# IntelLabs/bayesian-torch

Hardware: AMD Instinct MI355X
Metric: MC-samples/sec (Bayesian-ResNet18, 224^2, bs=64) (higher is better)
Workload: dtype bf16

## Files before the change

### bayesian_torch_amd/csrc/btx_api.hip

```cpp
#include <hip/hip_runtime.h>
#include <math.h>
#include <string.h>
#include "../../include/btx.h"
#include <stdlib.h>
#include "btx_contract.h"
#include "btx_rng.h"
#include "btx_presample.h"

using namespace btx;

static int contract_fwd_impl(int kind, const BtxGeom* g, const void* x, const float* mu_w, const float* rho_w,
                             const float* mu_b, const float* rho_b, void* out, const BtxRng* rng, const BtxNoise* noise,
                             int act_dtype, int prec, uint32_t flags, void* ws, size_t ws_bytes, void* stream,
                             const BtxEpilogue* ep, const BtxLanes* ln) {
  if (!g || !x || !mu_w || !rho_w || !out || !rng) return BTX_E_NULL;
  const int lanes = ln ? ln->n : 1;
  if ((mu_b == nullptr) != (rho_b == nullptr)) return BTX_E_NULL;
  const uintptr_t al = (uintptr_t)x | (uintptr_t)mu_w | (uintptr_t)rho_w | (uintptr_t)out |
                       (uintptr_t)(noise && noise->eps_w ? noise->eps_w : nullptr) |
                       (uintptr_t)(ep && ep->residual ? ep->residual : nullptr);
  FwdSel sel;
  int rc = select_fwd(kind, g, act_dtype, prec, flags, (al & 15) != 0, noise, ep, &sel);
  if (rc) return rc;
  const Plan& pl = sel.pl;
// ... 48 lines not shown
  {
    const long long in_elems = (long long)g->NB * g->D * g->H * g->W * g->C;
    const long long xb = in_elems * (act_dtype == BTX_ACT_BF16 ? 2 : 4), wb = (long long)g->N * pl.K * 4;
    p.x_bytes = xb < 0xffffffffLL ? (uint32_t)xb : 0xffffffffu;
    p.w_bytes = wb < 0xffffffffLL ? (uint32_t)wb : 0xffffffffu;
  }

  p.fd_inner = make_fastdiv((uint32_t)(pl.ntiles * g->groups * pl.ksplits)); p.fd_ksplits = make_fastdiv((uint32_t)pl.ksplits);
  p.fd_ntiles = make_fastdiv((uint32_t)pl.ntiles); p.fd_rtiles = make_fastdiv(1u);
  p.fd_mtiles = make_fastdiv((uint32_t)(pl.mtiles > 0 ? pl.mtiles : 1));
  {
    const double w_b = (prec == BTX_PREC_BF16 ? 2.0 : 4.0) * (double)g->N * pl.K * (kind == BTX_KIND_FLIPOUT ? 2 : 1);
    p.wg_order = (uses_tiles(sel.family) && pl.mtiles > 1 && w_b >= WG_MAJOR_MIB * 1048576.0) ? 1 : 0;
  }
  p.fd_Wo = make_fastdiv((uint32_t)pl.Wo); p.fd_Ho = make_fastdiv((uint32_t)pl.Ho); p.fd_Do = make_fastdiv((uint32_t)pl.Do);
  if (uses_tiles(sel.family)) {
    p.wt = sampled_w ? (void*)sampled_w : (void*)((unsigned char*)ws + sel.wt_off);
    p.wt_ready = sampled_w ? 1 : 0;
    p.wt_bytes = (uint32_t)sel.wt_all;
    p.wt_delta_off = (uint32_t)sel.wt_one;
    p.lane_wt = (long long)sel.wt_one;
    p.lane_wt_delta = (kind == BTX_KIND_FLIPOUT) ? 1 : 0;
  }
  hipStream_t st = (hipStream_t)stream;
  typedef int (*LaunchFn)(int, const ContractParams&, int, hipStream_t);
  auto launch = [&](LaunchFn f32, LaunchFn bf16, LaunchFn x3) {
    return (prec == BTX_PREC_BF16 ? bf16 : prec == BTX_PREC_BF16X3 ? x3 : f32)(kind, p, pl.nwg * lanes, st);
  };
  switch (sel.family) {
    case BTX_FAMILY_STEM_POOL: {
      const StemPoolPlan& spp = sel.spp;
      p.pt_R = spp.PB; p.pt_rtiles = spp.bands; p.pt_Rp = spp.Rp; p.pt_astage = spp.astage; p.st_sbytes = spp.sbytes;
      p.pt_lds = spp.lds; p.pt_PP = spp.patch_bytes; p.sp_Hq = spp.Hq; p.sp_Wq = spp.Wq;
      p.fd_rtiles = make_fastdiv((uint32_t)spp.bands);
      rc = launch_stem_pool_bf16(kind, p, pl.nwg * lanes, st);
      break;
    }
    case BTX_FAMILY_STEM: {
      const StemPlan& stp = sel.stp;
      p.pt_R = stp.R; p.pt_Rp = stp.Rp; p.pt_rtiles = stp.rtiles; p.pt_nw = stp.nw; p.pt_astage = stp.astage;
      p.st_sbytes = stp.sbytes; p.pt_lds = stp.lds; p.pt_PP = stp.patch_bytes;
      p.fd_rtiles = make_fastdiv((uint32_t)stp.rtiles);
      rc = launch(launch_contract_stem_f32, launch_contract_stem_bf16, launch_contract_stem_x3);
      break;
    }
    case BTX_FAMILY_PATCH:
    case BTX_FAMILY_TAPS:
    case BTX_FAMILY_TAPS2: {
      const PatchPlan& pt = sel.pt;
      p.pt_G = pt.G; p.pt_R = pt.R; p.pt_Rp = pt.Rp; p.pt_Wp = pt.Wp; p.pt_PP = pt.PP; p.pt_NI = pt.NI;
      p.fd_ptWp = make_fastdiv((uint32_t)pt.Wp); p.fd_ptRp = make_fastdiv((uint32_t)pt.Rp); p.fd_ptR = make_fastdiv((uint32_t)pt.R);
      p.fd_rtiles = make_fastdiv((uint32_t)pt.rtiles);
      p.pt_rtiles = pt.rtiles; p.pt_nw = pt.nw; p.pt_astage = pt.astage; p.pt_lds = pt.lds;
      p.pt_taps = pt.taps; p.pt_kg = pt.kg; p.pt_lds_g = pt.lds_g;
      p.pt_wide = (pt.taps == 33 || pt.taps == 332) ? pt.wide : 0;
      if (p.pt_wide) {
        p.fd_ntiles = make_fastdiv((uint32_t)(pl.ntiles / 2));
        p.fd_inner = make_fastdiv((uint32_t)((pl.ntiles / 2) * g->groups * pl.ksplits));
      }
      p.pt_tall = pt.tall; p.pt_P = pt.P; p.pt_Wt = pt.Wt; p.pt_ncs = pt.ncs;
      p.fd_P = make_fastdiv((uint32_t)pt.P); p.fd_Wt = make_fastdiv((uint32_t)pt.Wt); p.fd_ncs = make_fastdiv((uint32_t)pt.ncs);
      rc = launch(launch_contract_patch_f32, launch_contract_patch_bf16, launch_contract_patch_x3);
      break;
    }
    case BTX_FAMILY_GEMM8:
      p.pt_rtiles = sel.g8_pairs;
// ... 139 lines not shown
```

### bayesian_torch_amd/csrc/btx_contract.h

```cpp
#pragma once
#include <hip/hip_runtime.h>
#include <stdint.h>
#include "btx_rng.h"
#include "btx_plan.h"

typedef __attribute__((ext_vector_type(8))) __bf16 bf16x8;
typedef __attribute__((ext_vector_type(4))) __bf16 bf16x4;
typedef __attribute__((ext_vector_type(4))) float f32x4;
typedef __attribute__((ext_vector_type(8))) float f32x8;
typedef __attribute__((ext_vector_type(16))) float f32x16;
typedef __attribute__((ext_vector_type(4))) uint32_t u32x4;
typedef __attribute__((ext_vector_type(2))) uint32_t u32x2;

namespace btx {

constexpr int NTHREADS = 512;
constexpr int ACTS_OFF = 0;
constexpr int SIGN_OFF = NG * BM * 16;
constexpr int WMU_OFF = SIGN_OFF + NG * BM * 4;
constexpr int WDL_OFF = WMU_OFF + NG * BN * 16;
constexpr int STAGE_BYTES = WDL_OFF + NG * BN * 16;
constexpr int LDS_BYTES = 2 * STAGE_BYTES;

struct FastDiv {
// ... 37 lines not shown
  int NB, D, H, W, C, Cg;
  int Do, Ho, Wo, N, Ng;
  int KD, KH, KW;
  int sd, sh, sw, pd, ph, pw, dd, dh, dw;
  int M, K;
  int mtiles, ntiles, groups, ksplits, kper;
  int transposed;
  int pointwise;
  uint32_t seed_lo, seed_hi, sample, layer;
  const uint32_t* sample_ptr;
  uint32_t kin_a, kin_b, kout_a, kout_b;
  const float* ep_scale;
  const float* ep_shift;
  const void* ep_res;
  int ep_relu;
  int out_bf16;
  int sign_unaligned;
  uint32_t x_bytes, w_bytes;
  int pt_G, pt_R, pt_Rp, pt_Wp, pt_PP, pt_NI, pt_rtiles;
  FastDiv fd_Wo, fd_Ho, fd_Do, fd_ptWp, fd_ptRp, fd_ptR;
  FastDiv fd_inner, fd_ksplits, fd_ntiles, fd_Cg, fd_KW, fd_KH, fd_rtiles;
  FastDiv fd_mtiles;
  int swap_signs;
  int par_major, par_Mq, par_Mqp, par_Hh, par_Wh;
  FastDiv fd_par_Mqp, fd_par_Hh, fd_par_Wh;
  FastDiv fd_sd, fd_sh, fd_sw;
  int wg_order;
  int pt_nw, pt_astage, pt_lds;
  int pt_kg;
  int pt_lds_g;
  int pt_taps;
  int pt_wide;
  int sp_Hq, sp_Wq;
  int st_sbytes;
  void* wt;
  uint32_t wt_bytes, wt_delta_off;
  int wt_ready;
  int pt_tall, pt_P, pt_Wt, pt_ncs;
  FastDiv fd_P, fd_Wt, fd_ncs;
  int lanes, lane_nwg;
  FastDiv fd_lane_nwg;
  long long lane_x, lane_out, lane_res, lane_wt, lane_partial;
  int lane_wt_delta;
  int reverse;
};

__device__ __forceinline__ uint32_t sample_word_scalar(const uint32_t* ptr) {
  return *(const __attribute__((address_space(4))) uint32_t*)(uintptr_t)ptr;
}

__device__ __forceinline__ int xcd_logical() {
  const int nwg = gridDim.x, L = blockIdx.x;
  const int q = nwg >> 3, r = nwg & 7, xcd = L & 7, slot = L >> 3;
  return (xcd < r ? xcd * (q + 1) : r * (q + 1) + (xcd - r) * q) + slot;
}

__device__ __forceinline__ ContractParams lane_view(const ContractParams& q, int& logical) {
  ContractParams p = q;
  if (q.reverse) logical = (int)gridDim.x - 1 - logical;
  if (q.lanes > 1) {
    uint32_t lane, loc;
    fdivmod((uint32_t)logical, q.fd_lane_nwg, (uint32_t)q.lane_nwg, lane, loc);
    logical = (int)loc;
    const long long l = (long long)lane;
    p.x = (const unsigned char*)q.x + l * q.lane_x;
    p.out = (unsigned char*)q.out + l * q.lane_out;
// ... 682 lines not shown
```

### bayesian_torch_amd/csrc/btx_contract_stempool.h

```cpp
#pragma once
#include <type_traits>
#include "btx_contract.h"
#include "btx_contract_dma.h"
#include "btx_epilogue.h"
#include "btx_mma.h"
#include "btx_presample.h"

namespace btx {

constexpr int SP_NB = 1;
constexpr int SP_HROWS = 2;
constexpr int SP_LROWS = 3;
constexpr int SP_MAXST = 7;

typedef __attribute__((ext_vector_type(8))) short i16x8;

template <bool RELU>
__device__ __forceinline__ u32x4 sp_max8(const u32x4 a, const u32x4 b) {
  if constexpr (RELU) {
    return __builtin_bit_cast(u32x4, __builtin_elementwise_max(__builtin_bit_cast(i16x8, a), __builtin_bit_cast(i16x8, b)));
  } else {
    u32x4 r;
#pragma unroll
    for (int d = 0; d < 4; ++d) {
// ... 28 lines not shown
      }
}

template <int KIND>
__global__ __launch_bounds__(512, 2) void stem_pool_kernel(const ContractParams pk) {
  int logical = xcd_logical();
  const ContractParams p = lane_view(pk, logical);
  constexpr int G = 8, BK = NG * G;
  extern __shared__ __attribute__((aligned(16))) unsigned char smem[];
#define SP_BARRIER() asm volatile("s_waitcnt lgkmcnt(0)\n\ts_barrier" ::: "memory")
  const RngLive rl = rng_live<KIND>(p);

  const int tid = threadIdx.x;
  int lane = tid & 63;
  int l31 = lane & 31;
  int h = lane >> 5;
  const int wave = __builtin_amdgcn_readfirstlane(tid >> 6);
  const int grp = wave >> 2, w4 = wave & 3;
  int gtid = tid & 255;

  uint32_t u_rest, u_ntile, u_img, u_band;
  fdivmod((uint32_t)logical, p.fd_ntiles, (uint32_t)p.ntiles, u_rest, u_ntile);
  fdivmod(u_rest, p.fd_rtiles, (uint32_t)p.pt_rtiles, u_img, u_band);
  const int ntile = (int)u_ntile, img = (int)u_img, band = (int)u_band;

  const int PB = p.pt_R;
  const int P0 = band * PB;
  const int c0 = 2 * P0 - 1;
  const int Hq = p.sp_Hq, Wq = p.sp_Wq, Wo = p.Wo, Ho = p.Ho;
  const int NH = min(PB, Hq - P0) + 1;
  const int RowE = p.W * p.C;
  const int nstages = p.K / BK;
  const int spr = p.Cg / BK;
  const int W_OFF = 0, A_OFF = nstages * DW_STAGE, X_OFF = A_OFF + 2 * p.pt_astage;
  const int S_OFF = X_OFF + (KIND == 1 ? p.pt_astage : 0), R_OFF = S_OFF + 2 * p.st_sbytes;
  const int row_b = Wo * 128;
  const int C_OFF = R_OFF + SP_HROWS * row_b;
  float* const ba_lds = (float*)(smem + R_OFF + SP_LROWS * row_b);
  const int NINF_OFF = R_OFF + SP_LROWS * row_b + 4 * BN * 4;
  if (threadIdx.x < 8) *(uint32_t*)(smem + NINF_OFF + 4 * threadIdx.x) = threadIdx.x < 4 ? 0x80008000u : 0xff80ff80u;

  const __amdgpu_buffer_rsrc_t x_rsrc = __builtin_amdgcn_make_buffer_rsrc((void*)p.x, 0, p.x_bytes, 0x00020000);
  const __amdgpu_buffer_rsrc_t wt_rsrc = __builtin_amdgcn_make_buffer_rsrc((void*)p.wt, 0, p.wt_bytes, 0x00020000);

  {
    constexpr int PER = (KIND == 1) ? 8 : 4;
    const uint32_t w_tile = (uint32_t)ntile * (uint32_t)(p.K / G) * 1024u + (uint32_t)lane * 16u;
    const int npc = nstages * PER;
    for (int i = wave; i < npc; i += 8) {
      const int st = i / PER, r = i % PER;
      const uint32_t src = w_tile + (uint32_t)st * (uint32_t)NG * 1024u + (uint32_t)(r & 3) * 1024u +
                           (r >= 4 ? p.wt_delta_off : 0u);
      dma16(wt_rsrc, src, smem + W_OFF + st * DW_STAGE + (r >= 4 ? 4096 : 0) + (r & 3) * 1024);
    }
  }
  auto tile_base_e = [&](int u) __attribute__((always_inline)) {
    return (img * p.H + (c0 + SP_HROWS * u) * p.sh) * RowE;
  };
  auto issue_patch = [&](int u, int wi, int nw) __attribute__((always_inline)) {
    const uint32_t base_b = (uint32_t)tile_base_e(u) * 2u;
    unsigned char* dst = smem + A_OFF + (u & 1) * p.pt_astage;
    const int npieces = p.pt_astage >> 10;
    for (int i = wi; i < npieces; i += nw) {
      const uint32_t o = (uint32_t)i * 1024u + (uint32_t)lane * 16u;
      dma16(x_rsrc, o < (uint32_t)p.pt_PP ? base_b + o : DMA_OOB, dst + i * 1024);
    }
  };
  auto write_signs = [&](int u, int ti, int nt) __attribute__((always_inline)) {
    if constexpr (KIND == 1) {
      const int word0 = tile_base_e(u) >> 5;
      const int nwords = p.st_sbytes >> 2;
      unsigned char* ss = smem + S_OFF + (u & 1) * p.st_sbytes;
      for (int w = ti; w < nwords; w += nt)
        *(uint32_t*)(ss + w * 4) = btx_sign_word((uint32_t)(word0 + w), rl.kin_a, rl.kin_b);
    }
  };
  auto build_signed = [&](int u) __attribute__((always_inline)) {
    if constexpr (KIND == 1) {
      const int base_e = tile_base_e(u);
      const int word0 = base_e >> 5;
      const unsigned char* raw = smem + A_OFF + (u & 1) * p.pt_astage;
      const unsigned char* ss = smem + S_OFF + (u & 1) * p.st_sbytes;
      unsigned char* dst = smem + X_OFF;
      const int nchunks = p.pt_PP >> 4;
      constexpr int SP_CPY = 5;
      if (nchunks <= SP_CPY * 256) {
        u32x4 v[SP_CPY];
        uint32_t w[SP_CPY];
        int ci[SP_CPY];
#pragma unroll
        for (int k = 0; k < SP_CPY; ++k) {
          ci[k] = min(gtid + 256 * k, nchunks - 1);
          v[k] = *(const u32x4*)(raw + ci[k] * 16);
          w[k] = *(const uint32_t*)(ss + (((base_e + 8 * ci[k]) >> 5) - word0) * 4);
        }
#pragma unroll
        for (int k = 0; k < SP_CPY; ++k) {
          const int e = base_e + 8 * ci[k];
          const uint32_t ws = w[k] << (((uint32_t)e >> 3 & 3u) * 4u);
#pragma unroll
          for (int d = 0; d < 4; ++d) v[k][d] ^= (ws << d) & 0x80008000u;
        }
#pragma unroll
        for (int k = 0; k < SP_CPY; ++k) *(u32x4*)(dst + ci[k] * 16) = v[k];
        return;
      }
      for (int i = gtid; i < nchunks; i += 256) {
        u32x4 v = *(const u32x4*)(raw + i * 16);
        const int e = base_e + 8 * i;
        const uint32_t w = *(const uint32_t*)(ss + ((e >> 5) - word0) * 4);
        const uint32_t ws = w << (((uint32_t)e >> 3 & 3u) * 4u);
#pragma unroll
        for (int d = 0; d < 4; ++d) v[d] ^= (ws << d) & 0x80008000u;
        *(u32x4*)(dst + i * 16) = v;
      }
    }
  };
  issue_patch(0, wave, 8);
  write_signs(0, tid, 512);
  {
    const bool has_bias = p.mu_b != nullptr;
    const bool has_aff = (p.ep_scale != nullptr) || (p.ep_shift != nullptr);
    ep_fill_constants<KIND>(p, rl, ba_lds, tid, ntile, 0, has_bias, has_aff);
  }
  const bool has_bias = p.mu_b != nullptr;
  const bool has_aff = (p.ep_scale != nullptr) || (p.ep_shift != nullptr);
  const bool relu = p.ep_relu != 0;

  int eo[2];
  int st_off[2];
  uint32_t st_orow[2];
#pragma unroll
  for (int mi = 0; mi < 2; ++mi) {
    const int pl = w4 * 64 + mi * 32 + l31;
    const bool ok = pl < 2 * Wo;
    const int plc = ok ? pl : 0;
    const int r = plc >= Wo ? 1 : 0;
    const int col = plc - r * Wo;
    eo[mi] = (r * p.sh * RowE + col * p.sw * p.C) * 2;
    st_off[mi] = ok ? R_OFF + r * row_b + col * 128 + (((col >> 1) & 7) << 4) + h * 8 : -1;
    st_orow[mi] = (uint32_t)(((img * Ho + c0 + r) * Wo + col) * p.N + ntile * BN);
  }
  int pool_coff[2][3];
#pragma unroll
  for (int j = 0; j < 2; ++j)
#pragma unroll
    for (int k = 0; k < 3; ++k) {
      const int pc = (gtid + 256 * j) >> 3, col = 2 * pc - 1 + k;
      pool_coff[j][k] = (pc < Wq && col >= 0 && col < Wo) ? col * 128 + (((gtid & 7) ^ ((col >> 1) & 7)) << 4) : -1;
    }
  int carry_off[4];
#pragma unroll
  for (int j = 0; j < 4; ++j) {
    const int col = (gtid + 256 * j) >> 3;
    carry_off[j] = col < Wo ? col * 128 + (((gtid & 7) ^ ((col >> 1) & 7)) << 4) : -1;
  }
  const __amdgpu_buffer_rsrc_t out_rsrc = __builtin_amdgcn_make_buffer_rsrc(
      p.out, 0, (uint32_t)((size_t)p.NB * Hq * Wq * p.N * 2), 0x00020000);

  f32x16 accm[2][2], accd[2][2];

  auto run_pass = [&](const unsigned char* abase, int woff, f32x16 (&acc)[2][2], int bs0, int bs1, auto mia_tag)
                      __attribute__((always_inline)) {
    constexpr int MIA = decltype(mia_tag)::value;
    int l_j = 0, l_row = 0, l_b = 0;
    auto advance_load = [&]() __attribute__((always_inline)) {
      l_b += BK * 2;
      if (++l_j == spr) { l_j = 0; l_row += RowE * 2; l_b = l_row; }
    };
    auto load = [&](SpFrag& f, int s) __attribute__((always_inline)) {
      const unsigned char* as = abase + l_b;
      const unsigned char* ws = smem + W_OFF + s * DW_STAGE + woff;
#pragma unroll
      for (int kk = 0; kk < NG / 2; ++kk) {
        const int row = 2 * kk + h;
#pragma unroll
        for (int mi = 0; mi < MIA; ++mi) f.a[kk][mi] = *(const u32x4*)(as + eo[mi] + row * 16);
#pragma unroll
        for (int ni = 0; ni < 2; ++ni) f.w[kk][ni] = *(const u32x4*)(ws + (row * BN + ni * 32 + l31) * 16);
      }
      advance_load();
    };
    int nb = 0;
    SpFrag fa, fb;
    load(fa, 0);
    auto iter = [&](int s, SpFrag& cur, SpFrag& nxt, auto zero_tag) __attribute__((always_inline)) {
      if (s == bs0 || s == bs1) { SP_BARRIER(); ++nb; }
      if (s + 1 < nstages) load(nxt, s + 1);
      sp_mma<MIA, decltype(zero_tag)::value>(cur, acc);
    };
    iter(0, fa, fb, std::true_type{});
    int s = 1;
    for (; s + 1 < nstages; s += 2) {
      iter(s, fb, fa, std::false_type{});
      iter(s + 1, fa, fb, std::false_type{});
    }
    if (s < nstages) iter(s, fb, fa, std::false_type{});
    return nb;
  };
  auto run_pass3 = [&](const unsigned char* abase, int woff, f32x16 (&acc)[2][2], int bs0, int bs1) __attribute__((always_inline)) {
    int l_j = 0, l_row = 0, l_b = 0, l_s = 0;
    auto req = [&](SpFrag& f, auto i_tag) __attribute__((always_inline)) {
      constexpr int i = decltype(i_tag)::value, kk = i >> 2, j = i & 3;
      const int row = 2 * kk + h;
      if constexpr (j < 2) f.a[kk][j] = *(const u32x4*)(abase + l_b + eo[j] + row * 16);
      else f.w[kk][j - 2] = *(const u32x4*)(smem + W_OFF + l_s * DW_STAGE + woff + (row * BN + (j - 2) * 32 + l31) * 16);
    };
    auto advance = [&]() __attribute__((always_inline)) {
      ++l_s;
      l_b += BK * 2;
      if (++l_j == spr) { l_j = 0; l_row += RowE * 2; l_b = l_row; }
    };
    auto mma_half = [&](const SpFrag& f, auto kk_tag, auto zero_tag) __attribute__((always_inline)) {
      constexpr int kk = decltype(kk_tag)::value;
      constexpr bool ZERO = decltype(zero_tag)::value;
#pragma unroll
      for (int mi = 0; mi < 2; ++mi)
#pragma unroll
        for (int ni = 0; ni < 2; ++ni) {
          const f32x16 zc = {0.f, 0.f, 0.f, 0.f, 0.f, 0.f, 0.f, 0.f, 0.f, 0.f, 0.f, 0.f, 0.f, 0.f, 0.f, 0.f};
          acc[mi][ni] = __builtin_amdgcn_mfma_f32_32x32x16_bf16(__builtin_bit_cast(bf16x8, f.w[kk][ni]),
                                                               __builtin_bit_cast(bf16x8, f.a[kk][mi]),
                                                               (ZERO && kk == 0) ? zc : acc[mi][ni], 0, 0, 0);
        }
    };
    using I0 = std::integral_constant<int, 0>;
    using I1 = std::integral_constant<int, 1>;
    int nb = 0;
    auto stage = [&](SpFrag& cur, SpFrag& pre, int s_, auto zero_tag) __attribute__((always_inline)) {
      if (s_ == bs0 || s_ == bs1) { SP_BARRIER(); ++nb; }
      __builtin_amdgcn_s_waitcnt(0xc07f | (8 << 8));
      __builtin_amdgcn_sched_barrier(0);
      static_for_ep<0, 7>([&](auto i_tag) __attribute__((always_inline)) { req(pre, i_tag); });
      __builtin_amdgcn_sched_barrier(0);
      mma_half(cur, I0{}, zero_tag);
      __builtin_amdgcn_sched_barrier(0);
      __builtin_amdgcn_s_waitcnt(0xc07f | (14 << 8));
      __builtin_amdgcn_sched_barrier(0);
      req(pre, std::integral_constant<int, 7>{});
      advance();
      __builtin_amdgcn_sched_barrier(0);
      mma_half(cur, I1{}, zero_tag);
      __builtin_amdgcn_sched_barrier(0);
    };
    SpFrag f0, f1, f2;
    static_for_ep<0, 8>([&](auto i_tag) __attribute__((always_inline)) { req(f0, i_tag); });
    advance();
    __builtin_amdgcn_sched_barrier(0);
    static_for_ep<0, 7>([&](auto i_tag) __attribute__((always_inline)) { req(f1, i_tag); });
    __builtin_amdgcn_sched_barrier(0);
    __builtin_amdgcn_s_waitcnt(0xc07f | (14 << 8));
    __builtin_amdgcn_sched_barrier(0);
    req(f1, std::integral_constant<int, 7>{});
    advance();
    __builtin_amdgcn_sched_barrier(0);
    stage(f0, f2, 0, std::true_type{});
    for (int s_ = 1; s_ < nstages; s_ += 3) {
      stage(f1, f0, s_, std::false_type{});
      stage(f2, f1, s_ + 1, std::false_type{});
      stage(f0, f2, s_ + 2, std::false_type{});
    }
    return nb;
  };
  auto run_k = [&](int u, auto mia_tag) __attribute__((always_inline)) {
    const unsigned char* raw = smem + A_OFF + (u & 1) * p.pt_astage;
    int nb;
    __builtin_amdgcn_s_setprio(2);
    if constexpr (KIND == 1) {
      if (decltype(mia_tag)::value == 2 && (nstages - 1) % 3 == 0) run_pass3(raw, 0, accm, -1, -1);
      else run_pass(raw, 0, accm, -1, -1, mia_tag);
      SP_BARRIER();
      run_pass(smem + X_OFF, 4096, accd, -1, -1, mia_tag);
      nb = SP_NB;
    } else {
      const int b0_ = (nstages * 4 + 3) / 7 > 0 ? (nstages * 4 + 3) / 7 : -1, b1_ = -1;
      if (decltype(mia_tag)::value == 2 && (nstages - 1) % 3 == 0) nb = run_pass3(raw, 0, accm, b0_, b1_);
      else nb = run_pass(raw, 0, accm, b0_, b1_, mia_tag);
    }
    for (; nb < SP_NB; ++nb) SP_BARRIER();
    __builtin_amdgcn_s_setprio(0);
  };

  auto stage_half = [&](int u, int mia, auto ni_tag, auto bias_tag, auto aff_tag, auto m0_tag, auto m1_tag) __attribute__((always_inline)) {
    constexpr int ni = decltype(ni_tag)::value;
    constexpr bool BIAS = decltype(bias_tag)::value, AFF = decltype(aff_tag)::value;
    constexpr int TM0 = decltype(m0_tag)::value, TM1 = decltype(m1_tag)::value;
    uint32_t SB = 0x80000000u;
    asm volatile("" : "+s"(SB));
    uint32_t wsh[2] = {0u, 0u};
    if constexpr (KIND == 1) {
#pragma unroll
      for (int mi = 0; mi < 2; ++mi) {
        const uint32_t orow = st_orow[mi] + (uint32_t)(SP_HROWS * u * Wo * p.N);
        wsh[mi] = btx_sign_word((orow + 32u * ni) >> 5, rl.kout_a, rl.kout_b) << (2 * h);
      }
    }
    bool wr[2];
#pragma unroll
    for (int mi = 0; mi < 2; ++mi) wr[mi] = mi < mia && st_off[mi] >= 0;
    f32x4 bm_[4], bd_[4], sc_[4], sh_[4];
#pragma unroll
    for (int q = 0; q < 4; ++q) {
      const int cl = ni * 32 + 8 * q + 4 * h;
      if constexpr (BIAS) {
        bm_[q] = *(const f32x4*)(ba_lds + cl);
        bd_[q] = *(const f32x4*)(ba_lds + BN + cl);
      }
      if constexpr (AFF) {
        sc_[q] = *(const f32x4*)(ba_lds + 2 * BN + cl);
        sh_[q] = *(const f32x4*)(ba_lds + 3 * BN + cl);
      }
    }
#pragma unroll
// ... 73 lines not shown
      l0[j] = *(const u32x4*)(smem + ((in && r0_ok) ? R_OFF + carry_off[j] : NI_OFF));
      l1[j] = *(const u32x4*)(smem + ((in && r1_ok) ? R_OFF + row_b + carry_off[j] : NI_OFF));
    }
#pragma unroll
    for (int j = 0; j < 4; ++j) cnew[j] = sp_max8<RL>(l0[j], l1[j]);
  };
  auto write_carry = [&](const u32x4 (&cnew)[4]) __attribute__((always_inline)) {
#pragma unroll
    for (int j = 0; j < 4; ++j)
      if (carry_off[j] >= 0) *(u32x4*)(smem + C_OFF + carry_off[j]) = cnew[j];
  };
  auto clear_acc = [&](int mi0) __attribute__((always_inline)) {
#pragma unroll
    for (int a = 0; a < 2; ++a)
      if (a >= mi0) {
#pragma unroll
        for (int b = 0; b < 2; ++b)
#pragma unroll
          for (int r = 0; r < 16; ++r) { accm[a][b][r] = 0.f; accd[a][b][r] = 0.f; }
      }
  };
  auto mia_of = [&](int u) __attribute__((always_inline)) {
    const int limit = (u == NH - 1) ? Wo : 2 * Wo;
    const int m = (limit - w4 * 64 + 31) >> 5;
    return m < 0 ? 0 : (m > 2 ? 2 : m);
  };

  u32x4 cnew[4] = {{0u, 0u, 0u, 0u}, {0u, 0u, 0u, 0u}, {0u, 0u, 0u, 0u}, {0u, 0u, 0u, 0u}};
  bool carry_pending = false;
  asm volatile("s_waitcnt vmcnt(0)" ::: "memory");
  SP_BARRIER();
  using T = std::true_type;
  using F = std::false_type;
  for (int ph = 0; ph <= NH; ++ph) {
    asm volatile("" : "+v"(lane), "+v"(l31), "+v"(h), "+v"(gtid), "+v"(eo[0]), "+v"(eo[1]), "+v"(st_off[0]), "+v"(st_off[1]));
    asm volatile("" : "+v"(st_orow[0]), "+v"(st_orow[1]), "+v"(carry_off[0]), "+v"(carry_off[1]), "+v"(carry_off[2]),
                      "+v"(carry_off[3]));
    asm volatile("" : "+v"(pool_coff[0][0]), "+v"(pool_coff[0][1]), "+v"(pool_coff[0][2]), "+v"(pool_coff[1][0]),
                      "+v"(pool_coff[1][1]), "+v"(pool_coff[1][2]));
    if (grp == (ph & 1)) {
      if (carry_pending) { write_carry(cnew); carry_pending = false; }
      if (ph < NH) {
        if (ph + 1 < NH) issue_patch(ph + 1, w4, 4);
        build_signed(ph);
        const int mia = mia_of(ph);
        if (mia == 2) run_k(ph, std::integral_constant<int, 2>{});
        else if (mia == 1) { clear_acc(1); run_k(ph, std::integral_constant<int, 1>{}); }
        else { clear_acc(0); for (int b_ = 0; b_ < SP_NB; ++b_) SP_BARRIER(); }
        asm volatile("s_waitcnt vmcnt(0)" ::: "memory");
      } else {
        clear_acc(0);
        for (int b_ = 0; b_ < SP_NB; ++b_) SP_BARRIER();
      }
    } else {
      const int u = ph - 1;
      if (ph + 1 < NH) write_signs(ph + 1, gtid, 256);
      if (u >= 0) {
        const int mia = mia_of(u);
        stage_dispatch(u, mia, std::integral_constant<int, 0>{});
        stage_dispatch(u, mia, std::integral_constant<int, 1>{});
        SP_BARRIER();
        if (relu) pool_all(u, cnew, T{}); else pool_all(u, cnew, F{});
        carry_pending = true;
      } else {
        for (int b_ = 0; b_ < SP_NB; ++b_) SP_BARRIER();
      }
    }
    SP_BARRIER();
  }
}
#undef SP_BARRIER

static int launch_stem_pool_impl(int kind, const ContractParams& p, int nwg, hipStream_t st) {
#define BTX_LAUNCH_SP(KIND)                                                                                       \
  do {                                                                                                            \
    auto kfn = stem_pool_kernel<KIND>;                                                                            \
    static bool attr_done = false;                                                                                \
    if (!attr_done) {                                                                                             \
      hipError_t e = hipFuncSetAttribute((const void*)kfn, hipFuncAttributeMaxDynamicSharedMemorySize, 163840);   \
      if (e != hipSuccess) return (int)e;                                                                         \
// ... 13 lines not shown
```

### bayesian_torch_amd/csrc/btx_plan.cpp

```cpp
#include <string.h>
#include "btx_plan.h"

namespace btx {

static inline long long plan_lanes(uint32_t flags) {
  const long long n = (flags >> BTX_FLAG_LANES_SHIFT) & 0xffu;
  return n > 1 ? n : 1;
}

static inline bool throughput_plan(uint32_t flags) { return (flags & BTX_FLAG_CONCURRENT) || plan_lanes(flags) > 1; }

static int split_k(long long base1, int units, int unit_cost, int max_split, bool full_splits, bool throughput, bool short_exit) {
  int ks = 1;
  long long best = -1;
  for (int c = 1; c <= max_split; ++c) {
    if (full_splits && units % c) continue;
    const int per = (units + c - 1) / c;
    const long long rounds = (base1 * c + SLOTS - 1) / SLOTS;
    const long long cost = rounds * (per * unit_cost + 4) + (c > 1 ? 1 : 0);
    if (best < 0 || cost < best) { best = cost; ks = c; }
    if (throughput && (base1 * c >= 64 || (short_exit && base1 * c >= 16 && per <= 16))) { ks = c; break; }
  }
  return ks;
}
// ... 203 lines not shown
    for (; R >= 1; --R) {
      const long long Rp = (long long)(R - 1) * g->sh + g->KH;
      const long long pb = Rp * rowB;
      const long long astage = (pb + 1023) / 1024 * 1024;
      const long long sbytes = ((pb / esz + 31) / 32 + 3) * 4;
      const long long sb16 = (sbytes + 15) / 16 * 16;
      if (astage + sb16 > cap) continue;
      long long lds = astage + sb16 + PT_WD * 8192;
      const long long ep = (long long)nw * PT_EP_WAVE + 1024;
      if (lds < ep) lds = ep;
      st->R = R; st->Rp = (int)Rp; st->rtiles = (pl.Ho + R - 1) / R; st->nw = nw; st->astage = (int)astage;
      st->sbytes = (int)sb16; st->lds = (int)lds; st->patch_bytes = (int)pb;
      const long long nwg = (long long)g->NB * st->rtiles * pl.ntiles;
      if (nwg > 0x7fffffffLL) return false;
      st->nwg = (int)nwg;
      return true;
    }
  }
  return false;
}

static bool make_stem_pool_plan(const BtxGeom* g, int act_dtype, int prec, const Plan& pl, StemPoolPlan* sp, int lanes = 1) {
  if (prec != BTX_PREC_BF16 || act_dtype != BTX_ACT_BF16) return false;
  if (g->D != 1 || g->KD != 1 || pl.Do != 1 || g->groups != 1) return false;
  const int bk = NG * 8;
  if ((g->KW * g->C) % bk || pl.K % bk || (g->N % 64)) return false;
  const int nstages = pl.K / bk;
  if (nstages < 1 || nstages > 7) return false;
  if (2 * pl.Wo > 256 || pl.Ho < 1) return false;
  const int Hq = (pl.Ho - 1) / 2 + 1, Wq = (pl.Wo - 1) / 2 + 1;
  const long long rowB = (long long)g->W * g->C * 2;
  const long long Rp = (long long)g->sh + g->KH;
  const long long pb = Rp * rowB;
  const long long astage = (pb + 1023) / 1024 * 1024;
  const long long sbytes = ((pb / 2 + 31) / 32 + 3) * 4;
  const long long sb16 = (sbytes + 127) / 128 * 128;
  const long long lds = (long long)nstages * 8192 + 3 * astage + 2 * sb16 + 3LL * pl.Wo * 128 + 1024 + 64;
  if (lds > 163840) return false;
  const long long units = (long long)g->NB * pl.ntiles;
  long long PB = ((long long)Hq * units * (lanes > 1 ? lanes : 1)) / 256;
  if (PB < 4) PB = 4;
  if (PB > Hq) PB = Hq;
  const int bands = (Hq + (int)PB - 1) / (int)PB;
  const long long nwg = units * bands;
  if (nwg > 0x7fffffffLL) return false;
  sp->PB = (int)PB; sp->bands = bands; sp->Rp = (int)Rp; sp->astage = (int)astage; sp->sbytes = (int)sb16;
  sp->lds = (int)lds; sp->patch_bytes = (int)pb; sp->nwg = (int)nwg; sp->Hq = Hq; sp->Wq = Wq;
  return true;
}

size_t patch_wt_bytes(const Plan& pl, const BtxGeom* g, int kind, int prec, size_t* one, int lanes) {
  const size_t arr = (size_t)g->groups * pl.ntiles * 64 * (size_t)pl.K * (prec == BTX_PREC_BF16 ? 2 : 4);
  if (one) *one = arr;
  return arr * (size_t)(kind == BTX_KIND_FLIPOUT ? 1 + lanes : lanes);
}
static size_t pad256(size_t v) { return (v + 255) & ~(size_t)255; }

size_t plan_ws(const Plan& pl, const BtxGeom* g, int lanes) {
  return pl.ksplits > 1 ? (size_t)lanes * (size_t)pl.ksplits * (size_t)pl.M * (size_t)g->N * sizeof(float) : 0;
}

int select_fwd(int kind, const BtxGeom* g, int act_dtype, int prec, uint32_t flags, bool unaligned, const BtxNoise* noise,
               const BtxEpilogue* ep, FwdSel* s) {
  if (kind != BTX_KIND_REPARAM && kind != BTX_KIND_FLIPOUT) return BTX_E_UNSUPPORTED;
  if (act_dtype != BTX_ACT_F32 && act_dtype != BTX_ACT_BF16) return BTX_E_DTYPE;
  memset(s, 0, sizeof(*s));
  const int lanes = (int)plan_lanes(flags);
  Plan& pl = s->pl;
  int rc = make_plan(g, prec, flags, BM, &pl);
  if (rc) return rc;

  const int G = (prec == BTX_PREC_BF16) ? 8 : 4;
  const bool explicit_kloop = (flags & BTX_FLAG_GATHER) != 0;
  const bool gen = (pl.Cg % G != 0) || unaligned || explicit_kloop;
  const bool rowfuse = (flags & BTX_FLAG_ROWFUSE) != 0;
  bool dma = !gen && dma_shape_ok(g, act_dtype, prec, pl);
  {
    const bool pointwise_geom = !(flags & BTX_FLAG_TRANSPOSED) && g->KD == 1 && g->KH == 1 && g->KW == 1 && g->sd == 1 && g->sh == 1 &&
                                g->sw == 1 && g->pd == 0 && g->ph == 0 && g->pw == 0;
    if (dma && !rowfuse && pointwise_geom && lanes == 1 && !(flags & BTX_FLAG_CONCURRENT) && pl.M <= 256 && prec != BTX_PREC_BF16X3 &&
// ... 212 lines not shown
```

### bayesian_torch_amd/csrc/btx_plan.h

```cpp
#pragma once
#include <stddef.h>
#include <stdint.h>
#include "../../include/btx.h"

namespace btx {

constexpr int BM = 256;
constexpr int BN = 64;
constexpr int NG = 4;
constexpr int DBM = 512;

constexpr int PT_WD = 4;
constexpr int PT_EP_ROW = 272;
constexpr int PT_EP_WAVE = 64 * PT_EP_ROW;
constexpr int PT_MAXNI = 8;

constexpr long long SLOTS = 256;
constexpr double TALL_MIN_GAIN = 1.15;
constexpr int GEMM8_MIN_K = 128;
constexpr double WG_MAJOR_MIB = 3.0;

struct Plan {
  int Do, Ho, Wo, Cg, Ng, M, K, mtiles, ntiles, ksplits, kper, nwg;
};

struct PatchPlan {
  int G, R, Rp, Wp, PP, NI, rtiles, nw, astage, lds;
  int taps, kg, lds_g;
  int wide;
  int tall, P, Wt, ncs;
};

struct StemPlan {
  int R, Rp, rtiles, nw, astage, sbytes, lds, patch_bytes, nwg;
};

struct StemPoolPlan {
  int PB, bands, Rp, astage, sbytes, lds, patch_bytes, nwg, Hq, Wq;
};

struct FwdSel {
  int family;
  Plan pl;
  int par_major;
  int par_mqp, g8_pairs, out_bf16;
  StemPlan stp;
  StemPoolPlan spp;
  PatchPlan pt;
  size_t need, wt_off, wt_one, wt_all;
};
static inline bool uses_tiles(int family) { return family >= BTX_FAMILY_DMA; }

int select_fwd(int kind, const BtxGeom* g, int act_dtype, int prec, uint32_t flags, bool unaligned, const BtxNoise* noise,
               const BtxEpilogue* ep, FwdSel* s);

int make_plan(const BtxGeom* g, int prec, uint32_t flags, int bm, Plan* pl);
size_t plan_ws(const Plan& pl, const BtxGeom* g, int lanes = 1);
size_t patch_wt_bytes(const Plan& pl, const BtxGeom* g, int kind, int prec, size_t* one, int lanes = 1);

}
```

Baseline: 2034.

## Use a row ring buffer in stem-pool kernel to reuse overlapping input rows

The fused stem+maxpool kernel used to reload the full input patch (Rp rows) for every pair of output rows into double-buffered LDS stages. It now keeps a circular LDS ring of input rows and DMAs only the newly needed 2*sh rows per phase. Sign building for flipout is likewise limited to the new rows. The A-fragment addressing walks the ring with wraparound per kernel row. This cuts redundant global loads and sign XOR work and reduces LDS footprint. The cost is extra address arithmetic in the inner loop and more complex plan constraints.

Result: faster. 2058 (median of 6 runs) (+1.2%).

```diff
diff --git a/bayesian_torch_amd/csrc/btx_api.hip b/bayesian_torch_amd/csrc/btx_api.hip
--- a/bayesian_torch_amd/csrc/btx_api.hip
+++ b/bayesian_torch_amd/csrc/btx_api.hip
@@ -104,6 +104,7 @@
       const StemPoolPlan& spp = sel.spp;
       p.pt_R = spp.PB; p.pt_rtiles = spp.bands; p.pt_Rp = spp.Rp; p.pt_astage = spp.astage; p.st_sbytes = spp.sbytes;
       p.pt_lds = spp.lds; p.pt_PP = spp.patch_bytes; p.sp_Hq = spp.Hq; p.sp_Wq = spp.Wq;
+      p.sp_ring = spp.ring; p.sp_ring0 = spp.ring0;
       p.fd_rtiles = make_fastdiv((uint32_t)spp.bands);
       rc = launch_stem_pool_bf16(kind, p, pl.nwg * lanes, st);
       break;
diff --git a/bayesian_torch_amd/csrc/btx_contract.h b/bayesian_torch_amd/csrc/btx_contract.h
--- a/bayesian_torch_amd/csrc/btx_contract.h
+++ b/bayesian_torch_amd/csrc/btx_contract.h
@@ -93,6 +93,7 @@
   int pt_taps;
   int pt_wide;
   int sp_Hq, sp_Wq;
+  int sp_ring, sp_ring0;
   int st_sbytes;
   void* wt;
   uint32_t wt_bytes, wt_delta_off;
diff --git a/bayesian_torch_amd/csrc/btx_contract_stempool.h b/bayesian_torch_amd/csrc/btx_contract_stempool.h
--- a/bayesian_torch_amd/csrc/btx_contract_stempool.h
+++ b/bayesian_torch_amd/csrc/btx_contract_stempool.h
@@ -84,8 +84,12 @@
   const int RowE = p.W * p.C;
   const int nstages = p.K / BK;
   const int spr = p.Cg / BK;
-  const int W_OFF = 0, A_OFF = nstages * DW_STAGE, X_OFF = A_OFF + 2 * p.pt_astage;
-  const int S_OFF = X_OFF + (KIND == 1 ? p.pt_astage : 0), R_OFF = S_OFF + 2 * p.st_sbytes;
+  const int RowB = RowE * 2;
+  const int RingB = p.sp_ring * RowB;
+  const int AdvB = SP_HROWS * p.sh * RowB;
+  const int KeepB = p.pt_PP - AdvB;
+  const int W_OFF = 0, A_OFF = nstages * DW_STAGE, X_OFF = A_OFF + p.pt_astage;
+  const int S_OFF = X_OFF + p.pt_astage, R_OFF = S_OFF + 2 * p.st_sbytes;
   const int row_b = Wo * 128;
   const int C_OFF = R_OFF + SP_HROWS * row_b;
   float* const ba_lds = (float*)(smem + R_OFF + SP_LROWS * row_b);
@@ -109,53 +113,62 @@
   auto tile_base_e = [&](int u) __attribute__((always_inline)) {
     return (img * p.H + (c0 + SP_HROWS * u) * p.sh) * RowE;
   };
-  auto issue_patch = [&](int u, int wi, int nw) __attribute__((always_inline)) {
-    const uint32_t base_b = (uint32_t)tile_base_e(u) * 2u;
-    unsigned char* dst = smem + A_OFF + (u & 1) * p.pt_astage;
-    const int npieces = p.pt_astage >> 10;
+  auto new_base_e = [&](int u) __attribute__((always_inline)) {
+    return tile_base_e(u) + (u ? (KeepB >> 1) : 0);
+  };
+  auto issue_rows = [&](int u, int pos, int wi, int nw) __attribute__((always_inline)) {
+    const uint32_t base_b = (uint32_t)new_base_e(u) * 2u;
+    const uint32_t nbytes = (uint32_t)(u ? AdvB : p.pt_PP);
+    unsigned char* dst = smem + A_OFF + pos;
+    const int npieces = (int)((nbytes + 1023u) >> 10);
     for (int i = wi; i < npieces; i += nw) {
       const uint32_t o = (uint32_t)i * 1024u + (uint32_t)lane * 16u;
-      dma16(x_rsrc, o < (uint32_t)p.pt_PP ? base_b + o : DMA_OOB, dst + i * 1024);
+      dma16(x_rsrc, o < nbytes ? base_b + o : DMA_OOB, dst + i * 1024);
     }
   };
   auto write_signs = [&](int u, int ti, int nt) __attribute__((always_inline)) {
     if constexpr (KIND == 1) {
-      const int word0 = tile_base_e(u) >> 5;
-      const int nwords = p.st_sbytes >> 2;
+      const int word0 = new_base_e(u) >> 5;
+      const int nwords = u ? min(p.st_sbytes >> 2, (((AdvB >> 1) + 31) >> 5) + 1) : p.st_sbytes >> 2;
       unsigned char* ss = smem + S_OFF + (u & 1) * p.st_sbytes;
       for (int w = ti; w < nwords; w += nt)
         *(uint32_t*)(ss + w * 4) = btx_sign_word((uint32_t)(word0 + w), rl.kin_a, rl.kin_b);
     }
   };
-  auto build_signed = [&](int u) __attribute__((always_inline)) {
+  auto build_signed = [&](int u, int pos) __attribute__((always_inline)) {
     if constexpr (KIND == 1) {
-      const int base_e = tile_base_e(u);
+      const int base_e = new_base_e(u);
       const int word0 = base_e >> 5;
-      const unsigned char* raw = smem + A_OFF + (u & 1) * p.pt_astage;
+      const unsigned char* raw = smem + A_OFF + pos;
       const unsigned char* ss = smem + S_OFF + (u & 1) * p.st_sbytes;
-      unsigned char* dst = smem + X_OFF;
-      const int nchunks = p.pt_PP >> 4;
-      constexpr int SP_CPY = 5;
-      if (nchunks <= SP_CPY * 256) {
-        u32x4 v[SP_CPY];
-        uint32_t w[SP_CPY];
-        int ci[SP_CPY];
-#pragma unroll
-        for (int k = 0; k < SP_CPY; ++k) {
+      unsigned char* dst = smem + X_OFF + pos;
+      const int nchunks = (u ? AdvB : p.pt_PP) >> 4;
+      auto copy = [&](auto n_tag) __attribute__((always_inline)) {
+        constexpr int N = decltype(n_tag)::value;
+        u32x4 v[N];
+        uint32_t w[N];
+        int ci[N];
+#pragma unroll
+        for (int k = 0; k < N; ++k) {
           ci[k] = min(gtid + 256 * k, nchunks - 1);
           v[k] = *(const u32x4*)(raw + ci[k] * 16);
           w[k] = *(const uint32_t*)(ss + (((base_e + 8 * ci[k]) >> 5) - word0) * 4);
         }
 #pragma unroll
-        for (int k = 0; k < SP_CPY; ++k) {
+        for (int k = 0; k < N; ++k) {
           const int e = base_e + 8 * ci[k];
           const uint32_t ws = w[k] << (((uint32_t)e >> 3 & 3u) * 4u);
 #pragma unroll
           for (int d = 0; d < 4; ++d) v[k][d] ^= (ws << d) & 0x80008000u;
         }
 #pragma unroll
-        for (int k = 0; k < SP_CPY; ++k) *(u32x4*)(dst + ci[k] * 16) = v[k];
-        return;
+        for (int k = 0; k < N; ++k) *(u32x4*)(dst + ci[k] * 16) = v[k];
+      };
+      if (u == 0) {
+        if (nchunks <= 5 * 256) { copy(std::integral_constant<int, 5>{}); return; }
+      } else {
+        if (nchunks <= 2 * 256) { copy(std::integral_constant<int, 2>{}); return; }
+        if (nchunks <= 3 * 256) { copy(std::integral_constant<int, 3>{}); return; }
       }
       for (int i = gtid; i < nchunks; i += 256) {
         u32x4 v = *(const u32x4*)(raw + i * 16);
@@ -168,7 +181,7 @@
       }
     }
   };
-  issue_patch(0, wave, 8);
+  issue_rows(0, p.sp_ring0 * RowB, wave, 8);
   write_signs(0, tid, 512);
   {
     const bool has_bias = p.mu_b != nullptr;
@@ -180,6 +193,7 @@
   const bool relu = p.ep_relu != 0;
 
   int eo[2];
+  int rm[2];
   int st_off[2];
   uint32_t st_orow[2];
 #pragma unroll
@@ -189,7 +203,8 @@
     const int plc = ok ? pl : 0;
     const int r = plc >= Wo ? 1 : 0;
     const int col = plc - r * Wo;
-    eo[mi] = (r * p.sh * RowE + col * p.sw * p.C) * 2;
+    eo[mi] = col * p.sw * p.C * 2 + h * 16;
+    rm[mi] = -r;
     st_off[mi] = ok ? R_OFF + r * row_b + col * 128 + (((col >> 1) & 7) << 4) + h * 8 : -1;
     st_orow[mi] = (uint32_t)(((img * Ho + c0 + r) * Wo + col) * p.N + ntile * BN);
   }
@@ -212,13 +227,29 @@
 
   f32x16 accm[2][2], accd[2][2];
 
-  auto run_pass = [&](const unsigned char* abase, int woff, f32x16 (&acc)[2][2], int bs0, int bs1, auto mia_tag)
+  auto ring_walk_start = [&](int sb, int& l_r0, int& l_r1) __attribute__((always_inline)) {
+    l_r0 = sb;
+    l_r1 = sb + p.sh * RowB;
+    if (l_r1 >= RingB) l_r1 -= RingB;
+  };
+  auto ring_walk_advance = [&](int& l_j, int& l_r0, int& l_r1, int& l_b, int& l_d, auto spr1_tag) __attribute__((always_inline)) {
+    const bool next_row = decltype(spr1_tag)::value || (l_j + 1 == spr);
+    const int n0 = l_r0 + RowB >= RingB ? 0 : l_r0 + RowB;
+    const int n1 = l_r1 + RowB >= RingB ? 0 : l_r1 + RowB;
+    l_j = next_row ? 0 : l_j + 1;
+    l_r0 = next_row ? n0 : l_r0;
+    l_r1 = next_row ? n1 : l_r1;
+    l_b = next_row ? n0 : l_b + BK * 2;
+    l_d = l_r1 - l_r0;
+  };
+  auto run_pass = [&](const unsigned char* abase, int sb, int woff, f32x16 (&acc)[2][2], int bs0, int bs1, auto mia_tag, auto spr1_tag)
                       __attribute__((always_inline)) {
     constexpr int MIA = decltype(mia_tag)::value;
-    int l_j = 0, l_row = 0, l_b = 0;
+    int l_j = 0, l_r0, l_r1;
+    ring_walk_start(sb, l_r0, l_r1);
+    int l_b = l_r0, l_d = l_r1 - l_r0;
     auto advance_load = [&]() __attribute__((always_inline)) {
-      l_b += BK * 2;
-      if (++l_j == spr) { l_j = 0; l_row += RowE * 2; l_b = l_row; }
+      ring_walk_advance(l_j, l_r0, l_r1, l_b, l_d, spr1_tag);
     };
     auto load = [&](SpFrag& f, int s) __attribute__((always_inline)) {
       const unsigned char* as = abase + l_b;
@@ -227,7 +258,7 @@
       for (int kk = 0; kk < NG / 2; ++kk) {
         const int row = 2 * kk + h;
 #pragma unroll
-        for (int mi = 0; mi < MIA; ++mi) f.a[kk][mi] = *(const u32x4*)(as + eo[mi] + row * 16);
+        for (int mi = 0; mi < MIA; ++mi) f.a[kk][mi] = *(const u32x4*)(as + (eo[mi] + (rm[mi] & l_d)) + kk * 32);
 #pragma unroll
         for (int ni = 0; ni < 2; ++ni) f.w[kk][ni] = *(const u32x4*)(ws + (row * BN + ni * 32 + l31) * 16);
       }
@@ -250,18 +281,19 @@
     if (s < nstages) iter(s, fb, fa, std::false_type{});
     return nb;
   };
-  auto run_pass3 = [&](const unsigned char* abase, int woff, f32x16 (&acc)[2][2], int bs0, int bs1) __attribute__((always_inline)) {
-    int l_j = 0, l_row = 0, l_b = 0, l_s = 0;
+  auto run_pass3 = [&](const unsigned char* abase, int sb, int woff, f32x16 (&acc)[2][2], int bs0, int bs1, auto spr1_tag) __attribute__((always_inline)) {
+    int l_j = 0, l_r0, l_r1, l_s = 0;
+    ring_walk_start(sb, l_r0, l_r1);
+    int l_b = l_r0, l_d = l_r1 - l_r0;
     auto req = [&](SpFrag& f, auto i_tag) __attribute__((always_inline)) {
       constexpr int i = decltype(i_tag)::value, kk = i >> 2, j = i & 3;
       const int row = 2 * kk + h;
-      if constexpr (j < 2) f.a[kk][j] = *(const u32x4*)(abase + l_b + eo[j] + row * 16);
+      if constexpr (j < 2) f.a[kk][j] = *(const u32x4*)(abase + l_b + (eo[j] + (rm[j] & l_d)) + kk * 32);
       else f.w[kk][j - 2] = *(const u32x4*)(smem + W_OFF + l_s * DW_STAGE + woff + (row * BN + (j - 2) * 32 + l31) * 16);
     };
     auto advance = [&]() __attribute__((always_inline)) {
       ++l_s;
-      l_b += BK * 2;
-      if (++l_j == spr) { l_j = 0; l_row += RowE * 2; l_b = l_row; }
+      ring_walk_advance(l_j, l_r0, l_r1, l_b, l_d, spr1_tag);
     };
     auto mma_half = [&](const SpFrag& f, auto kk_tag, auto zero_tag) __attribute__((always_inline)) {
       constexpr int kk = decltype(kk_tag)::value;
@@ -314,23 +346,27 @@
     }
     return nb;
   };
-  auto run_k = [&](int u, auto mia_tag) __attribute__((always_inline)) {
-    const unsigned char* raw = smem + A_OFF + (u & 1) * p.pt_astage;
+  auto run_k_spr = [&](int sb, auto mia_tag, auto spr1_tag) __attribute__((always_inline)) {
+    const unsigned char* raw = smem + A_OFF;
     int nb;
     __builtin_amdgcn_s_setprio(2);
     if constexpr (KIND == 1) {
-      if (decltype(mia_tag)::value == 2 && (nstages - 1) % 3 == 0) run_pass3(raw, 0, accm, -1, -1);
-      else run_pass(raw, 0, accm, -1, -1, mia_tag);
+      if (decltype(mia_tag)::value == 2 && (nstages - 1) % 3 == 0) run_pass3(raw, sb, 0, accm, -1, -1, spr1_tag);
+      else run_pass(raw, sb, 0, accm, -1, -1, mia_tag, spr1_tag);
       SP_BARRIER();
-      run_pass(smem + X_OFF, 4096, accd, -1, -1, mia_tag);
+      run_pass(smem + X_OFF, sb, 4096, accd, -1, -1, mia_tag, spr1_tag);
       nb = SP_NB;
     } else {
       const int b0_ = (nstages * 4 + 3) / 7 > 0 ? (nstages * 4 + 3) / 7 : -1, b1_ = -1;
-      if (decltype(mia_tag)::value == 2 && (nstages - 1) % 3 == 0) nb = run_pass3(raw, 0, accm, b0_, b1_);
-      else nb = run_pass(raw, 0, accm, b0_, b1_, mia_tag);
+      if (decltype(mia_tag)::value == 2 && (nstages - 1) % 3 == 0) nb = run_pass3(raw, sb, 0, accm, b0_, b1_, spr1_tag);
+      else nb = run_pass(raw, sb, 0, accm, b0_, b1_, mia_tag, spr1_tag);
     }
     for (; nb < SP_NB; ++nb) SP_BARRIER();
     __builtin_amdgcn_s_setprio(0);
+  };
+  auto run_k = [&](int sb, auto mia_tag) __attribute__((always_inline)) {
+    if (spr == 1) run_k_spr(sb, mia_tag, std::true_type{});
+    else run_k_spr(sb, mia_tag, std::false_type{});
   };
 
   auto stage_half = [&](int u, int mia, auto ni_tag, auto bias_tag, auto aff_tag, auto m0_tag, auto m1_tag) __attribute__((always_inline)) {
@@ -470,8 +506,10 @@
   SP_BARRIER();
   using T = std::true_type;
   using F = std::false_type;
-  for (int ph = 0; ph <= NH; ++ph) {
+  int sb = p.sp_ring0 * RowB;
+  for (int ph = 0; ph <= NH; ++ph, sb = sb + AdvB >= RingB ? sb + AdvB - RingB : sb + AdvB) {
     asm volatile("" : "+v"(lane), "+v"(l31), "+v"(h), "+v"(gtid), "+v"(eo[0]), "+v"(eo[1]), "+v"(st_off[0]), "+v"(st_off[1]));
+    asm volatile("" : "+v"(rm[0]), "+v"(rm[1]));
     asm volatile("" : "+v"(st_orow[0]), "+v"(st_orow[1]), "+v"(carry_off[0]), "+v"(carry_off[1]), "+v"(carry_off[2]),
                       "+v"(carry_off[3]));
     asm volatile("" : "+v"(pool_coff[0][0]), "+v"(pool_coff[0][1]), "+v"(pool_coff[0][2]), "+v"(pool_coff[1][0]),
@@ -479,11 +517,13 @@
     if (grp == (ph & 1)) {
       if (carry_pending) { write_carry(cnew); carry_pending = false; }
       if (ph < NH) {
-        if (ph + 1 < NH) issue_patch(ph + 1, w4, 4);
-        build_signed(ph);
+        const int nxt = sb + p.pt_PP >= RingB ? sb + p.pt_PP - RingB : sb + p.pt_PP;
+        const int cur = ph == 0 ? sb : (sb + KeepB >= RingB ? sb + KeepB - RingB : sb + KeepB);
+        if (ph + 1 < NH) issue_rows(ph + 1, nxt, w4, 4);
+        build_signed(ph, cur);
         const int mia = mia_of(ph);
-        if (mia == 2) run_k(ph, std::integral_constant<int, 2>{});
-        else if (mia == 1) { clear_acc(1); run_k(ph, std::integral_constant<int, 1>{}); }
+        if (mia == 2) run_k(sb, std::integral_constant<int, 2>{});
+        else if (mia == 1) { clear_acc(1); run_k(sb, std::integral_constant<int, 1>{}); }
         else { clear_acc(0); for (int b_ = 0; b_ < SP_NB; ++b_) SP_BARRIER(); }
         asm volatile("s_waitcnt vmcnt(0)" ::: "memory");
       } else {
diff --git a/bayesian_torch_amd/csrc/btx_plan.cpp b/bayesian_torch_amd/csrc/btx_plan.cpp
--- a/bayesian_torch_amd/csrc/btx_plan.cpp
+++ b/bayesian_torch_amd/csrc/btx_plan.cpp
@@ -259,10 +259,19 @@
   const long long rowB = (long long)g->W * g->C * 2;
   const long long Rp = (long long)g->sh + g->KH;
   const long long pb = Rp * rowB;
-  const long long astage = (pb + 1023) / 1024 * 1024;
+  const long long GR = 2LL * g->sh;
+  if (GR > Rp) return false;
+  const long long adv = GR * rowB;
+  const long long over_fill = (pb + 1023) / 1024 * 1024 - pb, over_adv = (adv + 1023) / 1024 * 1024 - adv;
+  const long long over = over_fill > over_adv ? over_fill : over_adv;
+  const long long dead = (over + rowB - 1) / rowB;
+  const long long NR = (Rp + GR + dead + GR - 1) / GR * GR;
+  const long long ring0 = (GR - Rp % GR) % GR;
+  const long long astage = (NR * rowB + 127) / 128 * 128;
+  if (astage < 1024) return false;
   const long long sbytes = ((pb / 2 + 31) / 32 + 3) * 4;
   const long long sb16 = (sbytes + 127) / 128 * 128;
-  const long long lds = (long long)nstages * 8192 + 3 * astage + 2 * sb16 + 3LL * pl.Wo * 128 + 1024 + 64;
+  const long long lds = (long long)nstages * 8192 + 2 * astage + 2 * sb16 + 3LL * pl.Wo * 128 + 1024 + 64;
   if (lds > 163840) return false;
   const long long units = (long long)g->NB * pl.ntiles;
   long long PB = ((long long)Hq * units * (lanes > 1 ? lanes : 1)) / 256;
@@ -273,6 +282,7 @@
   if (nwg > 0x7fffffffLL) return false;
   sp->PB = (int)PB; sp->bands = bands; sp->Rp = (int)Rp; sp->astage = (int)astage; sp->sbytes = (int)sb16;
   sp->lds = (int)lds; sp->patch_bytes = (int)pb; sp->nwg = (int)nwg; sp->Hq = Hq; sp->Wq = Wq;
+  sp->ring = (int)NR; sp->ring0 = (int)ring0;
   return true;
 }
 
diff --git a/bayesian_torch_amd/csrc/btx_plan.h b/bayesian_torch_amd/csrc/btx_plan.h
--- a/bayesian_torch_amd/csrc/btx_plan.h
+++ b/bayesian_torch_amd/csrc/btx_plan.h
@@ -36,7 +36,7 @@
 };
 
 struct StemPoolPlan {
-  int PB, bands, Rp, astage, sbytes, lds, patch_bytes, nwg, Hq, Wq;
+  int PB, bands, Rp, astage, sbytes, lds, patch_bytes, nwg, Hq, Wq, ring, ring0;
 };
 
 struct FwdSel {
```
